# worm-privacy/proof-of-burn

Hardware: NVIDIA H100
Metric: main_proof_of_burn witnesses/sec (higher is better)
Workload: dtype u256 (BN254-Fr integer)

## Files before the change

proof-of-burn_b200/csrc/kernels.cuh:

```cuda
#pragma once
#include <cuda_runtime.h>
#include "vm_exec.h"
#include "cons_check.h"

using namespace pob;

namespace {

__constant__ uint64_t c_keccak_rc[24] = {
    0x0000000000000001ULL, 0x0000000000008082ULL, 0x800000000000808AULL, 0x8000000080008000ULL, 0x000000000000808BULL,
    0x0000000080000001ULL, 0x8000000080008081ULL, 0x8000000000008009ULL, 0x000000000000008AULL, 0x0000000000000088ULL,
    0x0000000080008009ULL, 0x000000008000000AULL, 0x000000008000808BULL, 0x800000000000008BULL, 0x8000000000008089ULL,
    0x8000000000008003ULL, 0x8000000000008002ULL, 0x8000000000000080ULL, 0x000000000000800AULL, 0x800000008000000AULL,
    0x8000000080008081ULL, 0x8000000000008080ULL, 0x0000000080000001ULL, 0x8000000080008008ULL};
__constant__ int c_keccak_rot[25] = {1, 10, 7, 11, 17, 18, 3, 5, 16, 8, 21, 24, 4, 15, 23, 19, 13, 12, 2, 20, 14, 22, 9, 6, 1};
__constant__ int c_keccak_inv_rot[25] = {0, 23, 17, 5, 11, 6, 22, 1, 8, 21, 0, 2, 16, 15, 19, 12, 7, 3, 4, 14, 18, 9, 20, 13, 10};

__device__ void absorb_warp(uint64_t *W, const AbsorbOp op) {
    const unsigned FULL = 0xffffffffu;
    const int lane = threadIdx.x & 31;
    const bool act = lane < 25;
    const int l = act ? lane : 0;
    uint64_t st = (act && op.s_idx != NONE_IDX) ? W[op.s_idx + l] : 0ull;
    if (lane < 17) st ^= W[op.blk_idx + lane];
// ... 219 lines not shown
                vm_exec_op(x, cur);
            }
        }
        for (uint32_t q = L.p_begin + gwarp; q < L.p_end; q += nwarp) poseidon_warp(x, a.poseidons[q], s_pk);
        { const uint32_t np = (L.p_end - L.p_begin) % nwarp, wv = (gwarp + nwarp - np) % nwarp;
          for (uint32_t w = L.w_begin + wv; w < L.w_end; w += nwarp) absorb_warp(U, a.absorbs[w]);
          const uint32_t nw2 = (np + (L.w_end - L.w_begin)) % nwarp, sv = (gwarp + nwarp - nw2) % nwarp;
          for (uint32_t q = L.s_begin + sv; q < L.s_end; q += nwarp) psum_warp(x, a.psums[q]); }
        if (inv_worker) {
            if (lv == a.ginv_level) {
                InvChain c;
                if (vm_ginv_start(x, a.ops, a.ginv_begin, a.inv_end, wid, NWK, c)) { inv_park(s_inv, INV_WORKERS, wt, c); inv_running = true; }
            } else if (inv_running) {
                InvChain c = inv_unpark(s_inv, INV_WORKERS, wt);
                if (inv_chain_steps(c, INV_STEPS)) { vm_ginv_finish(x, a.ops, a.ginv_begin, a.inv_end, wid, NWK, inv_chain_result(c)); inv_running = false; }
                else inv_park(s_inv, INV_WORKERS, wt, c);
            }
        }
        cluster_sync_all();
    }
    if (a.prof && inst == 0 && gt == 0) a.prof[a.n_levels] = clock64();
    if (inv_worker) {
        if (a.ginv_level >= a.n_levels) vm_inv_batch(x, a.ops, a.ginv_begin, a.inv_end, wid, NWK);
        else if (inv_running) {
            InvChain c = inv_unpark(s_inv, INV_WORKERS, wt);
            while (!inv_chain_steps(c, 64)) { }
            vm_ginv_finish(x, a.ops, a.ginv_begin, a.inv_end, wid, NWK, inv_chain_result(c));
        }
    }
    if (a.prof && inst == 0) { cluster_sync_all(); if (gt == 0) { a.prof[a.n_levels + 1] = clock64(); a.prof[a.n_levels + 2] = clock64(); } }
    __syncthreads();
    if (tid == 0 && s_status != STATUS_OK) atomicMin(a.status + inst, s_status);
    cluster_sync_all();
    if (gt == 0 && atomicAdd(a.status + inst, 0u) == STATUS_OK) a.status[inst] = 0u;
    for (uint32_t i = gt; i < a.n_outputs; i += GT) {
        uint64_t v[4]; vm_expand(a.out_codes[i], U, 0, a.val_base, a.konst, v);
        uint64_t *o = a.outputs + ((uint64_t)inst * a.n_outputs + i) * 4;
        o[0] = v[0]; o[1] = v[1]; o[2] = v[2]; o[3] = v[3];
    }
}

__device__ __forceinline__ void st128(uint64_t *p, uint64_t a, uint64_t b) { asm volatile("st.global.v2.b64 [%0], {%1, %2};" ::"l"(p), "l"(a), "l"(b)); }
__device__ __forceinline__ void st128cs(uint64_t *p, uint64_t a, uint64_t b) { asm volatile("st.global.cs.v2.b64 [%0], {%1, %2};" ::"l"(p), "l"(a), "l"(b)); }

struct ExpandArgs {
    const Tile *tiles; const Code *codes; const Fr *konst; const uint2 *round_desc;
    const uint64_t *stores; uint64_t store_stride; uint32_t val_base;
    uint64_t *const *wit;
    const uint32_t *inst;
    const uint32_t *status;
    uint32_t chunk_first;
    uint32_t tile0;
    uint32_t cs;
};

template <int T>
__global__ void __launch_bounds__(T) k_expand_round(const ExpandArgs a) {
    const uint32_t gi = a.inst[blockIdx.y];
    if (a.status[gi] != 0) return;
    const Tile t = a.tiles[blockIdx.x];
    const uint64_t *Ub = a.stores + (uint64_t)(gi - a.chunk_first) * a.store_stride + t.ubase;
    uint64_t *W = a.wit[blockIdx.y] + t.dst * 4;
    __shared__ __align__(16) uint2 sD[MAX_TILE_SIGNALS / 64];
    __shared__ __align__(16) uint64_t sWraw[ROUND_WORDS_SPAN + 3];
    __shared__ __align__(8) uint64_t s_bar;
    const uint32_t odd = (uint32_t)((reinterpret_cast<uintptr_t>(Ub) >> 3) & 1u);
    const uint32_t nd = (t.n + 63) >> 6, d_bytes = ((nd + 1) & ~1u) * 8u, w_bytes = (ROUND_WORDS_SPAN + 3) / 2 * 16u;
    if (threadIdx.x == 0) mbar_init(&s_bar, 1);
    __syncthreads();
    if (threadIdx.x == 0) {
        mbar_expect_tx(&s_bar, d_bytes + w_bytes);
        tma_load_1d(sD, a.round_desc + (t.code_off >> 6), d_bytes, &s_bar);
        tma_load_1d(sWraw, Ub - odd, w_bytes, &s_bar);
    }
    mbar_wait(&s_bar, 0);
    const uint64_t *sW = sWraw + odd;
#pragma unroll 8
    for (uint32_t u = threadIdx.x; u < 2 * t.n; u += T) {
        const uint32_t k = u >> 1;
        const uint2 d = sD[k >> 6];
        const uint32_t tt = k & 63, mode = d.y >> 16;
        uint32_t w = d.x & 0xffffu, b = tt;
        if (mode) {
            const uint32_t sidx = (mode - 1) * 64 + tt, g = sidx / 3, m = sidx - 3 * g;
            b = g; w = (m == 0) ? (d.x & 0xffffu) : (m == 1) ? (d.x >> 16) : (d.y & 0xffffu);
        }
        const uint64_t v = (u & 1u) ? 0ull : (sW[w] >> b) & 1ull;
        if (a.cs) st128cs(W + 2ull * u, v, 0); else st128(W + 2ull * u, v, 0);
    }
}

__global__ void __launch_bounds__(256, 3) k_expand_codes(const ExpandArgs a) {
    constexpr int UG = 4;
    const uint32_t gi = a.inst[blockIdx.x];
    if (a.status[gi] != 0) return;
    const Tile t = a.tiles[a.tile0 + blockIdx.y];
    const uint64_t *U = a.stores + (uint64_t)(gi - a.chunk_first) * a.store_stride;
    uint64_t *W = a.wit[blockIdx.x] + t.dst * 4;
    const uint64_t *Ub = U + t.ubase;
    __shared__ __align__(16) Code sC[TILE_SIGNALS + 4];
    __shared__ __align__(8) uint64_t s_bar;
    const uint32_t off4 = t.code_off & 3u, bytes = (((t.n + off4) * 4u) + 15u) & ~15u;
    if (threadIdx.x == 0) mbar_init(&s_bar, 1);
    __syncthreads();
    if (threadIdx.x == 0) { mbar_expect_tx(&s_bar, bytes); tma_load_1d(sC, a.codes + (t.code_off - off4), bytes, &s_bar); }
    mbar_wait(&s_bar, 0);
    const Code *c = sC + off4;
    const uint32_t n2 = 2 * t.n, h = threadIdx.x & 1u;
    for (uint32_t base = threadIdx.x; base < n2; base += 256 * UG) {
        uint64_t v[UG][2];
#pragma unroll
        for (int j = 0; j < UG; j++) {
            const uint32_t u = base + 256 * j;
            const Code cd = u < n2 ? c[u >> 1] : 0u;
            const uint32_t kind = code_kind(cd), p = code_payload(cd);
            v[j][0] = v[j][1] = 0;
            if (kind == K_VAL || kind == K_KONST) {
                const uint64_t *s = (kind == K_VAL) ? U + a.val_base + 4ull * p : reinterpret_cast<const uint64_t *>(a.konst + p);
                const ulonglong2 q = reinterpret_cast<const ulonglong2 *>(s)[h];
                v[j][0] = q.x; v[j][1] = q.y;
            } else if (!h) v[j][0] = (kind == K_BIT) ? (Ub[p >> 6] >> (p & 63)) & 1ull : p;
        }
#pragma unroll
        for (int j = 0; j < UG; j++) { const uint32_t u = base + 256 * j; if (u < n2) { if (a.cs) st128cs(W + 2ull * u, v[j][0], v[j][1]); else st128(W + 2ull * u, v[j][0], v[j][1]); } }
    }
}

__global__ void __launch_bounds__(256) k_digest(const uint64_t *wit, uint64_t n_signals, unsigned long long *out, const uint32_t *status) {
    if (status && *status != 0) return;
    uint64_t acc = 0;
    for (uint64_t i = (uint64_t)blockIdx.x * blockDim.x + threadIdx.x; i < n_signals; i += (uint64_t)gridDim.x * blockDim.x) {
        const ulonglong4 v = *reinterpret_cast<const ulonglong4 *>(wit + 4 * i);
        uint64_t h = (i + 1) * 0x9E3779B97F4A7C15ULL;
        h ^= v.x * 0xBF58476D1CE4E5B9ULL + v.y * 0x94D049BB133111EBULL + v.z * 0xD6E8FEB86659FD93ULL + v.w * 0xA0761D6478BD642FULL;
        h ^= h >> 29; h *= 0xBF58476D1CE4E5B9ULL; h ^= h >> 32;
        acc += h;
    }
    for (int o = 16; o > 0; o >>= 1) acc += __shfl_down_sync(0xffffffffu, acc, o);
    __shared__ uint64_t part[8];
    if ((threadIdx.x & 31) == 0) part[threadIdx.x >> 5] = acc;
    __syncthreads();
// ... 148 lines not shown
```

proof-of-burn_b200/csrc/pob_b200.cu:

```cuda
#include <cuda.h>
#include <cuda_runtime.h>
#include <fcntl.h>
#include <unistd.h>
#include <algorithm>
#include <chrono>
#include <condition_variable>
#include <cstdio>
#include <cstdlib>
#include <cstring>
#include <deque>
#include <mutex>
#include <stdexcept>
#include <string>
#include <thread>
#include <vector>
#include "../../include/pob_b200.h"
#include "compiler.h"
#include "kernels.cuh"
#include "ntt.cuh"
#include "r1cs.h"

using namespace pob;

static thread_local std::string g_err;
// ... 92 lines not shown
        busy[b] = true; next_b = (b + 1) % NB; return b;
    }
    void drain() { std::unique_lock<std::mutex> l(m); cv.wait(l, [this] { if (!q.empty()) return false; for (int i = 0; i < NB; i++) if (busy[i]) return false; return true; }); }
    static size_t header(uint8_t *o, uint64_t n) {
        uint32_t u32; uint64_t u64; Fr p = fr_p(); size_t k = 0;
        auto put = [&](const void *s, size_t b) { memcpy(o + k, s, b); k += b; };
        put("wtns", 4); u32 = 2; put(&u32, 4); u32 = 2; put(&u32, 4);
        u32 = 1; put(&u32, 4); u64 = 40; put(&u64, 8); u32 = 32; put(&u32, 4); put(p.l, 32); u32 = (uint32_t)n; put(&u32, 4);
        u32 = 2; put(&u32, 4); u64 = 32ull * n; put(&u64, 8);
        return k;
    }
    void send(const uint64_t *dwit, uint64_t n_signals, int fd) {
        CU(cudaSetDevice(device));
        if (fd >= 0) { uint8_t hd[80]; size_t hb = header(hd, n_signals); if (pwrite(fd, hd, hb, 0) != (ssize_t)hb) { std::lock_guard<std::mutex> l(m); io_err = true; } }
        const uint64_t total = 32ull * n_signals; const uint64_t nch = (total + bb - 1) / bb;
        for (uint64_t c = 0; c < nch; c++) {
            const uint64_t off = c * bb; const size_t bytes = (size_t)std::min<uint64_t>(bb, total - off);
            const int b = grab(); cudaStream_t s = cs[rr++ % NS];
            CU(cudaMemcpyAsync(buf[b], (const char *)dwit + off, bytes, cudaMemcpyDeviceToHost, s));
            CU(cudaEventRecord(ev[b], s));
            { std::lock_guard<std::mutex> l(m); q.push_back(Job{b, fd, 76 + off, bytes, c + 1 == nch}); }
            cv.notify_all();
            bytes_moved += bytes;
        }
        if (nch == 0 && fd >= 0) close(fd);
        for (int i = 1; i < NS; i++) { CU(cudaEventRecord(ev_join, cs[i])); CU(cudaStreamWaitEvent(cs[0], ev_join, 0)); }
    }
};

}

struct pob_handle {
    Program P; int device = 0; uint32_t n_sms = 0;
    Op *d_ops = nullptr; PsumOp *d_psums = nullptr; PoseidonOp *d_pos = nullptr; Fr *d_pos_konst = nullptr; AbsorbOp *d_abs = nullptr; Level *d_levels = nullptr; Code *d_aux = nullptr; Fr *d_konst = nullptr;
    Code *d_codes = nullptr; Tile *d_tiles = nullptr; Fr *d_invtab = nullptr; uint64_t *d_round_desc = nullptr;
    static const uint32_t RING = 2;
    uint32_t chunk = 0; uint64_t store_stride = 0; uint64_t *d_stores = nullptr; uint64_t *d_inputs = nullptr;
    std::vector<uint64_t *> slots;
    std::vector<VmSlot> slot_vm; size_t slot_bytes = 0; uint32_t n_compressed_slots = 0;
    std::vector<int64_t> slot_owner;
    std::vector<cudaEvent_t> slot_rel_ev; std::vector<uint8_t> slot_rel_pending;
    std::vector<uint32_t> last_status; uint32_t last_n = 0;
    uint32_t cap_n = 0; uint32_t *d_status = nullptr; uint64_t *d_outputs = nullptr; unsigned long long *d_digests = nullptr;
    uint64_t **d_witptr = nullptr; uint32_t *d_planinst = nullptr;
    uint32_t *h_status = nullptr; uint64_t *h_outputs = nullptr; uint64_t *h_digests = nullptr; uint64_t **h_witptr = nullptr; uint32_t *h_planinst = nullptr;
    uint64_t *d_staged = nullptr; uint32_t n_staged = 0;
    long long *d_prof = nullptr; std::string prof_path;
    uint32_t xgroup = 0;
    uint32_t n_round_tiles = 0;
    uint64_t *d_block_base = nullptr; uint32_t n_blocks = 0;
    uint32_t round_dyn_smem = 85 * 1024;
    uint32_t codes_dyn_smem = 24 * 1024;
    uint32_t round_threads = 256, codes_overlap = 0; bool serialize = false;
    int eval_threads = 512; uint32_t eval_cluster = 0, eval_prefetch = 0;
    uint32_t pos_konst_bytes = 0, levels_bytes = 0, eval_smem = 0;
    bool skip_eval = false;
    uint32_t expand_cs = 0, eval_l2_mb = 0;
    cudaStream_t s_eval = nullptr, s_exp = nullptr, s_exp2 = nullptr, s_h2d = nullptr;
    cudaEvent_t ev_eval_done[RING] = {nullptr, nullptr}, ev_exp_done[RING] = {nullptr, nullptr}, ev_h2d[RING] = {nullptr, nullptr},
                ev_start = nullptr, ev_end = nullptr, ev_tmp = nullptr, ev_fork = nullptr, ev_join = nullptr;
    std::vector<cudaEvent_t> ev_pool; size_t ev_used = 0;
    struct Group { uint32_t begin, end, chunk; cudaEvent_t t0, t1; };
    struct Batch {
        bool active = false, async = false, staged = false, expand = false, digest = false;
        const uint64_t *inputs = nullptr; uint32_t n = 0, nchunks = 0, next_eval = 0, next_group = 0, acq_pos = 0;
        std::vector<uint32_t> plan, slot;
        std::vector<uint8_t> st;
        std::vector<uint32_t> group_of;
        std::vector<Group> groups; std::vector<uint32_t> chunk_gend;
        std::vector<cudaEvent_t> e0, e1, est;
        pob_timing T{};
    } B;
    Exporter *exporter = nullptr;
    pob_timing timing{};
    struct DevCons {
        bool ready = false; ConsView flat{}, round{}; Fr *konst = nullptr; uint64_t *bases = nullptr; uint32_t n_blocks = 0;
        unsigned long long *rep = nullptr; std::vector<void *> allocs; pob_check_report info{};
    } cons, r1cs;
    struct DevNtt { bool ready = false; uint32_t log_n = 0; NttTables t{}; std::vector<void *> allocs; } ntt;
};

static void cons_info(const Program &P, pob_check_report *r) {
    memset(r, 0, sizeof *r);
    const uint64_t nb = P.round_block_sig.size();
    auto count = [&](const ConsSet &S, uint64_t mult) {
        r->n_constraints += mult * (S.eq.size() / 2 + S.kc.size());
        for (const ConsR1 &q : S.r1) { if (r1_hint(q)) r->n_hints += mult; else { r->n_constraints += mult; if (q.na) r->n_nonlinear += mult; } }
    };
    count(P.cons_flat, 1); count(P.cons_round, nb);
    std::vector<uint8_t> seen(P.n_signals, 0);
    auto mark = [&](const ConsSet &S, uint64_t base) {
        for (uint32_t i : S.eq) seen[base + i] = 1;
        for (const ConsTerm &t : S.kc) seen[base + t.idx] = 1;
        for (const ConsTerm &t : S.terms) if (t.idx != CONS_ONE) seen[base + t.idx] = 1;
    };
    mark(P.cons_flat, 0);
    for (uint64_t b : P.round_block_sig) mark(P.cons_round, b);
    for (uint8_t v : seen) r->signals_read += v;
    r->first_failed = ~0ull;
}
static ConsView upload_cons(pob_handle::DevCons &C, const ConsSet &S) {
    ConsView v{};
    auto up = [&](const void *src, size_t bytes) { void *d = nullptr; CU(cudaMalloc(&d, std::max<size_t>(16, bytes))); if (bytes) CU(cudaMemcpy(d, src, bytes, cudaMemcpyHostToDevice)); C.allocs.push_back(d); return d; };
    v.eq = (const uint32_t *)up(S.eq.data(), S.eq.size() * 4); v.n_eq = S.eq.size() / 2;
    v.kc = (const ConsTerm *)up(S.kc.data(), S.kc.size() * sizeof(ConsTerm)); v.n_kc = S.kc.size();
    v.r1 = (const ConsR1 *)up(S.r1.data(), S.r1.size() * sizeof(ConsR1)); v.n_r1 = S.r1.size();
// ... 60 lines not shown
    uint64_t *stores = h->d_stores + (size_t)r * E * h->store_stride;
    EvalArgs ea{h->d_ops, h->d_abs, h->d_pos, h->d_pos_konst, h->d_psums, h->d_levels, (uint32_t)P.levels.size(), P.inv_begin, P.ginv_begin, P.inv_end, h->d_aux, h->d_konst, h->d_invtab,
                h->d_codes + P.out_code_off, P.n_outputs, P.n_inputs, P.val_base, stores, h->store_stride, d_in,
                h->d_status + first, h->d_outputs + (size_t)first * no * 4, (c == 0) ? h->d_prof : nullptr, h->pos_konst_bytes, h->levels_bytes, h->eval_prefetch, P.ginv_level};
    CU(cudaEventRecord(B.e0[c], h->s_eval));
    {
        uint32_t C = h->eval_cluster;
        if (C == 0) { C = 8; while (C > 1 && cnt * C > h->n_sms) C >>= 1; }
        cudaLaunchConfig_t cfg{}; cudaLaunchAttribute at[1];
        cfg.gridDim = dim3(cnt * C); cfg.blockDim = dim3((unsigned)h->eval_threads); cfg.dynamicSmemBytes = h->eval_smem; cfg.stream = h->s_eval;
        at[0].id = cudaLaunchAttributeClusterDimension; at[0].val.clusterDim.x = C; at[0].val.clusterDim.y = 1; at[0].val.clusterDim.z = 1;
        cfg.attrs = at; cfg.numAttrs = 1;
        B.T.eval_clusters |= 1u << C;
        if (h->skip_eval && c >= R) CU(cudaMemsetAsync(h->d_status + first, 0, (size_t)cnt * 4, h->s_eval));
        else switch (h->eval_threads) {
        case 256: CU(cudaLaunchKernelEx(&cfg, k_eval<256>, ea)); break;
        case 512: CU(cudaLaunchKernelEx(&cfg, k_eval<512>, ea)); break;
        default: CU(cudaLaunchKernelEx(&cfg, k_eval<1024>, ea)); break;
        }
    }
    CU(cudaEventRecord(B.e1[c], h->s_eval));
    CU(cudaEventRecord(h->ev_eval_done[r], h->s_eval));
    B.T.eval_launches++;
    CU(cudaMemcpyAsync(h->h_status + first, h->d_status + first, (size_t)cnt * 4, cudaMemcpyDeviceToHost, h->s_eval));
    B.T.d2h_bytes += (uint64_t)cnt * 4;
    if (P.n_outputs) { CU(cudaMemcpyAsync(h->h_outputs + (size_t)first * no * 4, h->d_outputs + (size_t)first * no * 4, (size_t)cnt * no * 32, cudaMemcpyDeviceToHost, h->s_eval)); B.T.d2h_bytes += (uint64_t)cnt * no * 32; }
    CU(cudaEventRecord(B.est[c], h->s_eval));
    const uint32_t g0 = c ? B.chunk_gend[c - 1] : 0;
    if (B.chunk_gend[c] == g0) CU(cudaEventRecord(h->ev_exp_done[r], h->s_eval));
}

static void enqueue_group(pob_handle *h, uint32_t g) {
    pob_handle::Batch &B = h->B; const Program &P = h->P;
    const pob_handle::Group &G = B.groups[g];
    const uint32_t E = h->chunk, R = pob_handle::RING, r = G.chunk % R, gc = G.end - G.begin;
    CU(cudaStreamWaitEvent(h->s_exp, h->ev_eval_done[r], 0));
    for (uint32_t k = G.begin; k < G.end; k++) {
        const uint32_t s = B.slot[k];
        if (h->slot_rel_pending[s]) { CU(cudaStreamWaitEvent(h->s_exp, h->slot_rel_ev[s], 0)); h->slot_rel_pending[s] = 0; }
        h->slot_owner[s] = (int64_t)B.plan[k];
    }
    ExpandArgs xa{h->d_tiles, h->d_codes, h->d_konst, reinterpret_cast<const uint2 *>(h->d_round_desc), h->d_stores + (size_t)r * E * h->store_stride, h->store_stride, P.val_base,
                  h->d_witptr + G.begin, h->d_planinst + G.begin, h->d_status, G.chunk * E, 0, h->expand_cs};
    CU(cudaEventRecord(G.t0, h->s_exp));
    const uint32_t n_round = h->n_round_tiles, n_code = (uint32_t)P.tiles.size() - n_round;
    const bool fork = h->codes_overlap && n_round && n_code;
    cudaStream_t s_codes = fork ? h->s_exp2 : h->s_exp;
    auto launch_codes = [&]() {
        xa.tile0 = n_round;
        k_expand_codes<<<dim3(gc, n_code), 256, h->codes_dyn_smem, s_codes>>>(xa);
        B.T.other_launches++;
    };
    if (fork) { CU(cudaEventRecord(h->ev_fork, h->s_exp)); CU(cudaStreamWaitEvent(h->s_exp2, h->ev_fork, 0)); if (h->codes_overlap == 2) launch_codes(); }
    if (n_round) {
        xa.tile0 = 0;
        if (h->round_threads == 128) k_expand_round<128><<<dim3(n_round, gc), 128, h->round_dyn_smem, h->s_exp>>>(xa);
        else if (h->round_threads == 512) k_expand_round<512><<<dim3(n_round, gc), 512, h->round_dyn_smem, h->s_exp>>>(xa);
        else if (h->round_threads == 1024) k_expand_round<1024><<<dim3(n_round, gc), 1024, h->round_dyn_smem, h->s_exp>>>(xa);
        else k_expand_round<256><<<dim3(n_round, gc), 256, h->round_dyn_smem, h->s_exp>>>(xa);
    }
    if (n_code && !(fork && h->codes_overlap == 2)) launch_codes();
    if (fork) { CU(cudaEventRecord(h->ev_join, h->s_exp2)); CU(cudaStreamWaitEvent(h->s_exp, h->ev_join, 0)); }
    CU(cudaEventRecord(G.t1, h->s_exp));
    B.T.expand_launches++;
    if (B.digest) for (uint32_t k = G.begin; k < G.end; k++) {
        k_digest<<<h->n_sms * 8, 256, 0, h->s_exp>>>(h->slots[B.slot[k]], P.n_signals, h->d_digests + B.plan[k], h->d_status + B.plan[k]);
        B.T.other_launches++;
    }
    if (!B.async) for (uint32_t k = G.begin; k < G.end; k++) B.st[k] = 2;
    if (g + 1 == B.chunk_gend[G.chunk]) {
        CU(cudaEventRecord(h->ev_exp_done[r], h->s_exp));
        if (h->serialize) CU(cudaStreamWaitEvent(h->s_eval, h->ev_exp_done[r], 0));
    }
}

static bool group_slots_free(const pob_handle *h, uint32_t g) {
    const pob_handle::Batch &B = h->B; const uint32_t ns = (uint32_t)h->slots.size();
    for (uint32_t k = B.groups[g].begin; k < B.groups[g].end; k++) if (k >= ns && B.st[k - ns] != 2) return false;
    return true;
}
static void advance(pob_handle *h) {
    pob_handle::Batch &B = h->B; const uint32_t R = pob_handle::RING, ng = (uint32_t)B.groups.size();
    for (;;) {
        bool progressed = false;
        if (B.next_eval < B.nchunks && (B.next_eval < R || B.next_group >= B.chunk_gend[B.next_eval - R])) { enqueue_eval(h, B.next_eval++); progressed = true; }
        if (B.next_group < ng && B.groups[B.next_group].chunk < B.next_eval && group_slots_free(h, B.next_group)) { enqueue_group(h, B.next_group++); progressed = true; }
        if (!progressed) break;
    }
    CU(cudaGetLastError());
}

static int begin_batch(pob_handle *h, const uint64_t *inputs, uint32_t n, uint32_t flags, const uint32_t *retain, uint32_t n_retain, bool async, const char *who) {
    const bool staged = (flags & POB_RUN_INPUTS_STAGED) != 0, digest = (flags & POB_RUN_DIGEST) != 0;
    const bool expand = async || (flags & (POB_RUN_EXPAND | POB_RUN_DIGEST)) != 0 || retain != nullptr;
    if (h->B.active) return fail(POB_E_BUSY, std::string(who) + ": a batch is in flight on this handle (pob_finish it first)");
    if (staged ? (h->n_staged < n) : (inputs == nullptr && h->P.n_inputs)) return fail(POB_E_BAD_ARG, std::string(who) + ": no inputs");
    const uint32_t ns = (uint32_t)h->slots.size();
    if (retain) {
        if (n_retain > ns) return fail(POB_E_RANGE, std::string(who) + ": more retained instances than witness slots");
        for (uint32_t k = 0; k < n_retain; k++) if (retain[k] >= n || (k && retain[k] <= retain[k - 1])) return fail(POB_E_BAD_ARG, std::string(who) + ": retain[] must be strictly ascending instance indices");
    } else if (expand && !async && n > ns && !(flags & (POB_RUN_DIGEST | POB_RUN_DISCARD)))
        return fail(POB_E_RANGE, std::string(who) + ": n exceeds the resident witness slots; earlier witnesses would be overwritten unread -- use pob_submit/pob_acquire/pob_release, a retain list, POB_RUN_DIGEST or POB_RUN_DISCARD");
    CU(cudaSetDevice(h->device));
    ensure_batch_buffers(h, n);
    pob_handle::Batch &B = h->B;
    B = pob_handle::Batch();
    B.async = async; B.staged = staged; B.expand = expand; B.digest = digest; B.inputs = inputs; B.n = n;
    const uint32_t E = h->chunk;
    B.nchunks = (n + E - 1) / E;
    const uint32_t X = async ? std::max<uint32_t>(1, std::min(h->xgroup, ns / 2 ? ns / 2 : 1)) : h->xgroup;
    if (expand) {
        if (retain) B.plan.assign(retain, retain + n_retain);
// ... 18 lines not shown
    std::fill(h->slot_owner.begin(), h->slot_owner.end(), (int64_t)-1);
    std::fill(h->slot_rel_pending.begin(), h->slot_rel_pending.end(), (uint8_t)0);
    h->last_n = 0; h->last_status.clear();
    CU(cudaEventRecord(h->ev_start, h->s_eval));
    if (np) {
        CU(cudaMemcpyAsync(h->d_witptr, h->h_witptr, (size_t)np * sizeof(uint64_t *), cudaMemcpyHostToDevice, h->s_eval));
        CU(cudaMemcpyAsync(h->d_planinst, h->h_planinst, (size_t)np * 4, cudaMemcpyHostToDevice, h->s_eval));
    }
    if (digest) CU(cudaMemsetAsync(h->d_digests, 0, (size_t)n * 8, h->s_eval));
    CU(cudaEventRecord(h->ev_tmp, h->s_eval));
    CU(cudaStreamWaitEvent(h->s_h2d, h->ev_tmp, 0));
    B.active = true;
    advance(h);
    return POB_OK;
}

static int finish_batch(pob_handle *h, uint32_t *status, uint64_t *outputs, uint64_t *digests) {
    pob_handle::Batch &B = h->B; const Program &P = h->P;
    const uint32_t n = B.n; const size_t no = std::max<uint32_t>(1, P.n_outputs);
    for (auto &s : B.st) s = 2;
    advance(h);
    if (B.next_eval != B.nchunks || B.next_group != B.groups.size()) throw std::runtime_error("internal: batch did not drain");
    CU(cudaEventRecord(h->ev_tmp, h->s_eval));
    CU(cudaStreamWaitEvent(h->s_exp, h->ev_tmp, 0));
    if (B.digest) { CU(cudaMemcpyAsync(h->h_digests, h->d_digests, (size_t)n * 8, cudaMemcpyDeviceToHost, h->s_exp)); B.T.d2h_bytes += (uint64_t)n * 8; }
    CU(cudaEventRecord(h->ev_end, h->s_exp));
    CU(cudaStreamSynchronize(h->s_exp)); CU(cudaStreamSynchronize(h->s_eval)); CU(cudaStreamSynchronize(h->s_h2d));
    CU(cudaGetLastError());
    if (status) memcpy(status, h->h_status, (size_t)n * 4);
    if (outputs && P.n_outputs) memcpy(outputs, h->h_outputs, (size_t)n * no * 32);
    if (B.digest && digests) memcpy(digests, h->h_digests, (size_t)n * 8);
    pob_timing &T = B.T;
    CU(cudaEventElapsedTime(&T.total_ms, h->ev_start, h->ev_end));
    for (uint32_t c = 0; c < B.nchunks; c++) { float ms = 0; CU(cudaEventElapsedTime(&ms, B.e0[c], B.e1[c])); T.eval_ms += ms; }
    for (auto &G : B.groups) { float ms = 0; CU(cudaEventElapsedTime(&ms, G.t0, G.t1)); T.expand_ms += ms; }
    if (h->d_prof) {
        std::vector<long long> st(P.levels.size() + 3);
        CU(cudaMemcpy(st.data(), h->d_prof, st.size() * sizeof(long long), cudaMemcpyDeviceToHost));
        if (FILE *f = fopen(h->prof_path.c_str(), "w")) {
            for (size_t l = 0; l + 1 < st.size(); l++) {
                if (l < P.levels.size()) fprintf(f, "level %zu ops %u absorbs %u poseidons %u cycles %lld\n", l, P.levels[l].t_end - P.levels[l].t_begin, P.levels[l].w_end - P.levels[l].w_begin, P.levels[l].p_end - P.levels[l].p_begin, st[l + 1] - st[l]);
                else if (l == P.levels.size()) fprintf(f, "inverse-batch(table) ops %u cycles %lld\n", P.ginv_begin - P.inv_begin, st[l + 1] - st[l]);
                else fprintf(f, "inverse-batch(generic) ops %u cycles %lld\n", P.inv_end - P.ginv_begin, st[l + 1] - st[l]);
            }
            fclose(f);
        }
    }
    h->timing = T; h->last_n = n; h->last_status.assign(h->h_status, h->h_status + n);
    B.active = false;
    return POB_OK;
}
static void abort_batch(pob_handle *h) {
    cudaDeviceSynchronize(); cudaGetLastError();
    h->B.active = false; h->last_n = 0; h->last_status.clear();
    std::fill(h->slot_owner.begin(), h->slot_owner.end(), (int64_t)-1);
}

extern "C" {

const char *pob_last_error(void) { return g_err.c_str(); }
const char *pob_version(void) {
#ifdef POB_TUNING
    return "pob_b200 0.2 (sm_90a, TUNING build)";
#else
    return "pob_b200 0.2 (sm_90a)";
#endif
}

const char *pob_input_schema(const char *main_name, int *nparams) {
    if (!main_name) return nullptr;
    return main_input_schema(main_name, nparams);
}

int pob_layout_info(const char *main_name, const uint64_t *params, int nparams, int hcreate, pob_desc *out) {
    if (!main_name || !out || (nparams > 0 && !params)) return fail(POB_E_BAD_ARG, "pob_layout_info: null argument");
    try { Program P = compile_circuit(main_name, params_vec(params, nparams), flag_hcreate(hcreate), false, flag_opt(hcreate)); fill_desc(P, out); }
    catch (const std::exception &e) { return fail(POB_E_COMPILE, e.what()); }
    return POB_OK;
}

int pob_write_components(const char *main_name, const uint64_t *params, int nparams, int hcreate, const char *path, uint64_t *n_components) {
    if (!main_name || !path || (nparams > 0 && !params)) return fail(POB_E_BAD_ARG, "pob_write_components: null argument");
    try { uint64_t n = write_components(main_name, params_vec(params, nparams), flag_hcreate(hcreate), path); if (n_components) *n_components = n; }
    catch (const std::exception &e) { return fail(POB_E_COMPILE, e.what()); }
    return POB_OK;
}

int pob_write_r1cs(const char *main_name, const uint64_t *params, int nparams, int hcreate, const char *path, pob_r1cs_desc *out) {
    if (!main_name || !out || (nparams > 0 && !params)) return fail(POB_E_BAD_ARG, "pob_write_r1cs: null argument");
    try {
        const RowPlan R = build_row_plan(main_name, params_vec(params, nparams), flag_hcreate(hcreate), flag_opt(hcreate));
        memset(out, 0, sizeof *out);
        out->n_wires = R.n_wires; out->n_pub_out = R.n_outputs; out->n_pub_in = 0; out->n_prv_in = R.n_inputs; out->n_labels = R.n_labels;
        out->n_constraints = R.n_rows(); out->n_nonlinear = R.n_nonlinear; out->n_terms = R.n_terms; out->file_bytes = R.file_bytes();
        if (path) write_r1cs(R, path);
    } catch (const R1csIoError &e) { return fail(POB_E_IO, std::string("pob_write_r1cs: ") + e.what()); }
    catch (const std::exception &e) { return fail(POB_E_COMPILE, e.what()); }
    return POB_OK;
}

void pob_destroy(pob_handle *h) {
    if (!h) return;
    cudaSetDevice(h->device);
    delete h->exporter; h->exporter = nullptr;
    for (void *p : h->cons.allocs) cudaFree(p);
    for (void *p : h->r1cs.allocs) cudaFree(p);
    for (void *p : h->ntt.allocs) cudaFree(p);
    if (h->s_eval) cudaStreamSynchronize(h->s_eval);
    if (h->s_exp2) cudaStreamSynchronize(h->s_exp2);
    if (h->s_exp) cudaStreamSynchronize(h->s_exp);
    if (h->s_h2d) cudaStreamSynchronize(h->s_h2d);
    for (void *p : {(void *)h->d_ops, (void *)h->d_psums, (void *)h->d_pos, (void *)h->d_pos_konst, (void *)h->d_abs, (void *)h->d_levels, (void *)h->d_aux, (void *)h->d_konst, (void *)h->d_codes,
                    (void *)h->d_tiles, (void *)h->d_invtab, (void *)h->d_round_desc, (void *)h->d_stores, (void *)h->d_inputs, (void *)h->d_status,
                    (void *)h->d_outputs, (void *)h->d_digests, (void *)h->d_witptr, (void *)h->d_planinst, (void *)h->d_staged, (void *)h->d_prof, (void *)h->d_block_base})
        if (p) cudaFree(p);
    if (!h->slot_vm.empty()) {
        const DriverVmm &D = vmm();
        cudaDeviceSynchronize();
        for (const VmSlot &s : h->slot_vm) {
            if (s.mapped) D.unmap(s.va, h->slot_bytes);
            if (s.va) D.addressFree(s.va, h->slot_bytes);
            if (s.mem) D.release(s.mem);
        }
    }
    for (void *p : {(void *)h->h_status, (void *)h->h_outputs, (void *)h->h_digests, (void *)h->h_witptr, (void *)h->h_planinst}) if (p) cudaFreeHost(p);
    for (cudaEvent_t e : h->ev_pool) cudaEventDestroy(e);
    for (cudaEvent_t e : h->slot_rel_ev) cudaEventDestroy(e);
    for (uint32_t r = 0; r < pob_handle::RING; r++) {
        if (h->ev_eval_done[r]) cudaEventDestroy(h->ev_eval_done[r]);
        if (h->ev_exp_done[r]) cudaEventDestroy(h->ev_exp_done[r]);
        if (h->ev_h2d[r]) cudaEventDestroy(h->ev_h2d[r]);
    }
    for (cudaEvent_t e : {h->ev_start, h->ev_end, h->ev_tmp, h->ev_fork, h->ev_join}) if (e) cudaEventDestroy(e);
    for (cudaStream_t s : {h->s_h2d, h->s_eval, h->s_exp, h->s_exp2}) if (s) cudaStreamDestroy(s);
    delete h;
}

int pob_create(const char *main_name, const uint64_t *params, int nparams, int hcreate, int device, uint32_t max_slots, pob_handle **out) {
    if (!main_name || !out || (nparams > 0 && !params)) return fail(POB_E_BAD_ARG, "pob_create: null argument");
    *out = nullptr;
    int ndev = 0;
    if (cudaGetDeviceCount(&ndev) != cudaSuccess || ndev == 0) return fail(POB_E_NO_DEVICE, "pob_create: no CUDA device (this library has no CPU path)");
    if (device < 0 || device >= ndev) return fail(POB_E_NO_DEVICE, "pob_create: device index out of range");
    pob_handle *h = new pob_handle(); h->device = device;
    try { h->P = compile_circuit(main_name, params_vec(params, nparams), flag_hcreate(hcreate), false, flag_opt(hcreate)); }
    catch (const std::exception &e) { delete h; return fail(POB_E_COMPILE, e.what()); }
    try {
        const Program &P = h->P;
        CU(cudaSetDevice(device));
        { int v = 0; CU(cudaDeviceGetAttribute(&v, cudaDevAttrMultiProcessorCount, device)); h->n_sms = (uint32_t)v; }
        h->d_ops = upload(P.ops); h->d_psums = upload(P.psums); h->d_pos = upload(P.poseidons); h->d_pos_konst = upload(P.pos_konst); h->d_abs = upload(P.absorbs); h->d_levels = upload(P.levels); h->d_aux = upload(P.aux);
        h->pos_konst_bytes = (uint32_t)(P.pos_konst.size() * sizeof(Fr)); h->levels_bytes = (uint32_t)(std::max<size_t>(1, P.levels.size()) * sizeof(Level));
        h->d_konst = upload(P.konst);
        { std::vector<Code> cd = P.codes; cd.resize(cd.size() + 8, 0); h->d_codes = upload(cd); }
        if (const char *v = tune_env("POB_TILE_FILTER")) {
            std::vector<Tile> sub; for (const Tile &t : P.tiles) if ((atoi(v) == 1) == (t.pad != 0)) sub.push_back(t);
            h->P.tiles = sub;
        }
        h->d_tiles = upload(h->P.tiles);
        for (const Tile &t : h->P.tiles) if (t.pad) h->n_round_tiles++;
        { std::vector<uint64_t> bases; for (const Tile &t : P.tiles) if (t.pad && t.code_off == 0) bases.push_back(t.dst);
          std::sort(bases.begin(), bases.end()); h->n_blocks = (uint32_t)bases.size(); h->d_block_base = upload(bases); }
        h->d_invtab = upload(build_inverse_table());
        { std::vector<uint64_t> rd = P.round_desc; rd.resize(rd.size() + 2, 0); h->d_round_desc = upload(rd); }
        int pr_least = 0, pr_greatest = 0; CU(cudaDeviceGetStreamPriorityRange(&pr_least, &pr_greatest));
        CU(cudaStreamCreateWithPriority(&h->s_eval, cudaStreamNonBlocking, pr_greatest));
        CU(cudaStreamCreateWithPriority(&h->s_h2d, cudaStreamNonBlocking, pr_greatest));
// ... 24 lines not shown
        size_t gran = 0; CUD(D.granularity(&gran, &mprop, CU_MEM_ALLOC_GRANULARITY_RECOMMENDED));
        const size_t vbytes = (wbytes + gran - 1) / gran * gran;
        const uint64_t ring_bytes_per_inst = pob_handle::RING * (h->store_stride * 8 + (uint64_t)P.n_inputs * 32);
        uint64_t budget = (uint64_t)(free_b * 0.8);
        uint64_t nslots = budget > chunk * ring_bytes_per_inst ? (budget - chunk * ring_bytes_per_inst) / vbytes : 0;
        if (max_slots && nslots > max_slots) nslots = max_slots;
        if (nslots > 4096) nslots = 4096;
        if (nslots == 0) throw std::runtime_error("not even one witness slot fits in free HBM");
        h->chunk = chunk;
        CU(cudaMalloc(&h->d_stores, (size_t)pob_handle::RING * chunk * h->store_stride * 8));
        CU(cudaMalloc(&h->d_inputs, std::max<size_t>(32, (size_t)pob_handle::RING * chunk * P.n_inputs * 32)));
        h->slot_bytes = vbytes;
        CUmemAccessDesc acc{}; acc.location = mprop.location; acc.flags = CU_MEM_ACCESS_FLAGS_PROT_READWRITE;
        for (uint64_t s = 0; s < nslots; s++) {
            CUmemGenericAllocationHandle mem = 0;
            const CUresult r = D.create(&mem, vbytes, &mprop, 0);
            if (r == CUDA_ERROR_OUT_OF_MEMORY && s > 0) break;
            if (r == CUDA_ERROR_OUT_OF_MEMORY) throw std::runtime_error("not even one witness slot fits in free HBM (cuMemCreate)");
            if (r != CUDA_SUCCESS) throw std::runtime_error("cuMemCreate: CUresult " + std::to_string((int)r));
            h->slot_vm.push_back(VmSlot{}); VmSlot &m = h->slot_vm.back(); m.mem = mem;
            CUD(D.reserve(&m.va, vbytes, gran, 0, 0));
            CUD(D.map(m.va, vbytes, 0, m.mem, 0)); m.mapped = true;
            CUD(D.setAccess(m.va, vbytes, &acc, 1));
            CUmemAllocationProp got{}; CUD(D.properties(&got, m.mem));
            if (got.allocFlags.compressionType == CU_MEM_ALLOCATION_COMP_GENERIC) h->n_compressed_slots++;
            h->slots.push_back(reinterpret_cast<uint64_t *>(m.va));
        }
        nslots = h->slots.size();
        h->xgroup = (uint32_t)std::min<uint64_t>(std::min<uint64_t>(nslots, chunk), std::max<uint64_t>(16, (100ull << 30) / wbytes));
        if (const char *v = tune_env("POB_EVAL_THREADS")) h->eval_threads = atoi(v);
        if (const char *v = tune_env("POB_EVAL_CLUSTER")) h->eval_cluster = (uint32_t)std::max(0, std::min(8, atoi(v)));
        if (const char *v = tune_env("POB_EVAL_PREFETCH")) h->eval_prefetch = (uint32_t)(atoi(v) != 0);
        if (const char *v = tune_env("POB_SKIP_EVAL")) h->skip_eval = atoi(v) != 0;
        if (const char *v = tune_env("POB_EXPAND_CS")) h->expand_cs = (uint32_t)(atoi(v) != 0);
        if (const char *v = tune_env("POB_EVAL_L2_MB")) h->eval_l2_mb = (uint32_t)std::max(0, atoi(v));
        if (h->eval_threads != 256 && h->eval_threads != 512) h->eval_threads = 1024;
        h->eval_smem = h->pos_konst_bytes + h->levels_bytes + INV_WORKERS * INV_PARK_WORDS * 4u;
        if (h->eval_smem > 200 * 1024) throw std::runtime_error("the Poseidon constant table, the level table and the parked inversions do not fit in shared memory");
        CU(cudaFuncSetAttribute(k_eval<256>, cudaFuncAttributeMaxDynamicSharedMemorySize, (int)h->eval_smem));
        CU(cudaFuncSetAttribute(k_eval<512>, cudaFuncAttributeMaxDynamicSharedMemorySize, (int)h->eval_smem));
        CU(cudaFuncSetAttribute(k_eval<1024>, cudaFuncAttributeMaxDynamicSharedMemorySize, (int)h->eval_smem));
        if (const char *v = tune_env("POB_SERIALIZE")) h->serialize = atoi(v) != 0;
        if (const char *v = tune_env("POB_EXPAND_SMEM_KB")) h->round_dyn_smem = (uint32_t)atoi(v) * 1024u;
        if (const char *v = tune_env("POB_EXPAND_THREADS")) h->round_threads = (uint32_t)atoi(v);
        if (const char *v = tune_env("POB_CODES_OVERLAP")) h->codes_overlap = (uint32_t)atoi(v);
        if (const char *v = tune_env("POB_CODES_SMEM_KB")) h->codes_dyn_smem = (uint32_t)atoi(v) * 1024u;
        CU(cudaFuncSetAttribute(k_expand_codes, cudaFuncAttributeMaxDynamicSharedMemorySize, (int)h->codes_dyn_smem));
        if (h->round_dyn_smem > 48 * 1024) {
            CU(cudaFuncSetAttribute(k_expand_round<128>, cudaFuncAttributeMaxDynamicSharedMemorySize, (int)h->round_dyn_smem));
            CU(cudaFuncSetAttribute(k_expand_round<256>, cudaFuncAttributeMaxDynamicSharedMemorySize, (int)h->round_dyn_smem));
            CU(cudaFuncSetAttribute(k_expand_round<512>, cudaFuncAttributeMaxDynamicSharedMemorySize, (int)h->round_dyn_smem));
            CU(cudaFuncSetAttribute(k_expand_round<1024>, cudaFuncAttributeMaxDynamicSharedMemorySize, (int)h->round_dyn_smem));
        }
        if (const char *v = tune_env("POB_EXPAND_GROUP")) h->xgroup = (uint32_t)std::max(1, std::min<int>(atoi(v), (int)std::min<uint64_t>(nslots, chunk)));
        if (h->eval_l2_mb) {
            const size_t ring = (size_t)pob_handle::RING * chunk * h->store_stride * 8, carve = (size_t)h->eval_l2_mb << 20;
            CU(cudaDeviceSetLimit(cudaLimitPersistingL2CacheSize, carve));
            cudaDeviceProp prop; CU(cudaGetDeviceProperties(&prop, device));
            cudaStreamAttrValue av{};
            av.accessPolicyWindow.base_ptr = h->d_stores;
            av.accessPolicyWindow.num_bytes = std::min<size_t>(ring, (size_t)prop.accessPolicyMaxWindowSize);
            av.accessPolicyWindow.hitRatio = (float)std::min(1.0, (double)carve / (double)av.accessPolicyWindow.num_bytes);
            av.accessPolicyWindow.hitProp = cudaAccessPropertyPersisting; av.accessPolicyWindow.missProp = cudaAccessPropertyStreaming;
            CU(cudaStreamSetAttribute(h->s_eval, cudaStreamAttributeAccessPolicyWindow, &av));
        }
        h->slot_owner.assign(nslots, -1); h->slot_rel_pending.assign(nslots, 0);
        for (uint64_t s = 0; s < nslots; s++) { cudaEvent_t e; CU(cudaEventCreateWithFlags(&e, cudaEventDisableTiming)); h->slot_rel_ev.push_back(e); }
    } catch (const std::exception &e) {
        std::string m = e.what(); pob_destroy(h);
        return fail(m.find("slot") != std::string::npos ? POB_E_NO_MEMORY : POB_E_CUDA, "pob_create: " + m);
    }
    *out = h; return POB_OK;
}

int pob_witness_map(const pob_handle *h, uint32_t *map) {
    if (!h || !map) return fail(POB_E_BAD_ARG, "pob_witness_map: null argument");
    if (!h->P.opt_level) return fail(POB_E_BAD_ARG, "pob_witness_map: the handle produces the full --O0 witness (identity map)");
    memcpy(map, h->P.witness_map.data(), h->P.witness_map.size() * 4);
    return POB_OK;
}

int pob_describe(const pob_handle *h, pob_desc *out) {
    if (!h || !out) return fail(POB_E_BAD_ARG, "pob_describe: null argument");
    fill_desc(h->P, out); out->n_slots = (uint32_t)h->slots.size(); out->chunk = h->chunk; out->expand_group = h->xgroup;
    out->n_compressed_slots = h->n_compressed_slots; return POB_OK;
}

void *pob_alloc_pinned(uint64_t bytes) { void *p = nullptr; if (cudaMallocHost(&p, bytes ? bytes : 1) != cudaSuccess) { g_err = "cudaMallocHost failed"; return nullptr; } return p; }
void pob_free_pinned(void *p) { if (p) cudaFreeHost(p); }

int pob_stage_inputs(pob_handle *h, const uint64_t *inputs, uint32_t n) {
    if (!h || !inputs || n == 0) return fail(POB_E_BAD_ARG, "pob_stage_inputs: bad argument");
    if (h->B.active) return fail(POB_E_BUSY, "pob_stage_inputs: a batch is in flight");
    try {
        CU(cudaSetDevice(h->device));
        if (h->d_staged) { cudaFree(h->d_staged); h->d_staged = nullptr; h->n_staged = 0; }
        size_t bytes = std::max<size_t>(32, (size_t)n * h->P.n_inputs * 32);
        CU(cudaMalloc(&h->d_staged, bytes));
        if (h->P.n_inputs) CU(cudaMemcpy(h->d_staged, inputs, (size_t)n * h->P.n_inputs * 32, cudaMemcpyHostToDevice));
        h->n_staged = n;
    } catch (const std::exception &e) { return fail(POB_E_CUDA, e.what()); }
    return POB_OK;
}

static int run_batch_impl(pob_handle *h, const uint64_t *inputs, uint32_t n, uint32_t flags, const uint32_t *retain, uint32_t n_retain,
                          uint32_t *status, uint64_t *outputs, uint64_t *digests, const char *who) {
// ... 407 lines not shown
```

proof-of-burn_b200/csrc/program.h:

```cpp
#pragma once
#include <stdint.h>
#include <string>
#include <vector>
#include "fr_hd.h"

namespace pob {

typedef uint32_t Code;
enum : uint32_t { K_CONST = 0, K_BIT = 1, K_VAL = 2, K_KONST = 3 };
POB_HD uint32_t code_kind(Code c) { return c >> 30; }
POB_HD uint32_t code_payload(Code c) { return c & 0x3fffffffu; }
POB_HD Code c_const(uint32_t v) { return v; }
POB_HD Code c_bit(uint32_t u64idx, uint32_t bit) { return (1u << 30) | (u64idx << 6) | bit; }
POB_HD Code c_val(uint32_t slot) { return (2u << 30) | slot; }
POB_HD Code c_konst(uint32_t idx) { return (3u << 30) | idx; }
static const uint32_t MAX_STORE_U64 = 1u << 24;

enum Opc : uint32_t {
    OP_FMA = 1,
    OP_ISZ = 2,
    OP_INV = 3,
    OP_DIV = 4,
    OP_MOD = 5,
    OP_PACK8 = 6,
    OP_CHK_EQ = 7,
    OP_CHK_RANGE = 8,
    OP_GTC = 9,
    OP_SELSUM = 10,
};
struct Op { uint32_t opc_dst; Code a, b, c; };
POB_HD uint32_t op_opc(const Op &o) { return o.opc_dst >> 26; }
POB_HD uint32_t op_dst(const Op &o) { return o.opc_dst & 0x3ffffffu; }

static const uint32_t NONE_IDX = 0xffffffffu;
struct AbsorbOp { uint32_t s_idx, blk_idx, out_idx, pad; };
enum : uint32_t { RW = 238, RW_X5 = 25, RW_DD = 45, RW_TH = 65, RW_RP = 90, RW_CH = 162, RW_RC = 237, RW_OUT = 238,
                  ROUND_WORDS_SPAN = 263, ABSORB_WORDS = 25 + 24 * 238, ROUND_SIGNALS = 102656 };
POB_HD uint32_t rw_x5(int i, int k) { return RW_X5 + 4 * i + k; }
POB_HD uint32_t rw_dd(int i, int k) { return RW_DD + 4 * i + k; }
POB_HD uint32_t rw_th(int l) { return RW_TH + l; }
POB_HD uint32_t rw_rp(int i, int k) { return RW_RP + 3 * i + k; }
POB_HD uint32_t rw_ch(int l, int k) { return RW_CH + 3 * l + k; }
POB_HD uint32_t rw_out(int l) { return RW_OUT + l; }

struct PoseidonOp { uint32_t t, in_aux, base, koff, q0, q1; };
static const uint32_t POS_SEGMENTS = 16;
struct PosLayout { uint32_t t, rp, F1, PB, SB, LB, total, kC, kS, kM, kP, ktotal; };
POB_HD PosLayout pos_layout(uint32_t t) {
    PosLayout L; L.t = t; L.rp = (t == 3) ? 57u : (t == 4) ? 56u : 60u;
    L.F1 = t; L.PB = 21 * t; L.SB = L.PB + L.rp * (4 + t); L.LB = L.SB + 15 * t; L.total = L.LB + 3 * t + 1;
    L.kC = 0; L.kS = t * 8 + L.rp; L.kM = L.kS + L.rp * (2 * t - 1); L.kP = L.kM + t * t; L.ktotal = L.kP + t * t;
    return L;
}
POB_HD uint32_t pos_steps(const PosLayout &L) { return L.rp + 9; }
POB_HD uint32_t pos_state_off(const PosLayout &L, uint32_t q) {
    if (q == 0) return 0;
    if (q <= 4) return L.F1 + 5 * L.t * (q - 1) + 4 * L.t;
    if (q < 5 + L.rp) return L.PB + (q - 5) * (4 + L.t) + 4;
    return L.SB + 5 * L.t * (q - 5 - L.rp) + 4 * L.t;
}

POB_HD uint32_t pos_step_begin(const PosLayout &L, uint32_t q) {
    if (q == 0) return 0;
    if (q <= 4) return L.F1 + 5 * L.t * (q - 1);
    if (q < 5 + L.rp) return L.PB + (q - 5) * (4 + L.t);
    if (q < L.rp + 8) return L.SB + 5 * L.t * (q - 5 - L.rp);
    return q == L.rp + 8 ? L.LB : L.total;
}

struct PsumOp { uint32_t aux0, n, dst; Code x0; };

struct Level { uint32_t t_begin, t_end, w_begin, w_end, p_begin, p_end, s_begin, s_end; };

struct Tile { uint64_t dst; uint32_t n, code_off, ubase, pad; };
static const uint32_t TILE_SIGNALS = 8192;
static const uint32_t LAYOUT_TILE_SIGNALS = 4096;
static const uint32_t MAX_TILE_SIGNALS = 32768;

struct ConsTerm { uint32_t idx, coef; };
enum : uint32_t { CC_POS = 0, CC_NEG = 1, CC_KONST = 2, CC_RCBIT = 3 };
POB_HD uint32_t cc_kind(uint32_t c) { return c >> 30; }
POB_HD uint32_t cc_payload(uint32_t c) { return c & 0x3fffffffu; }
struct ConsR1 { uint32_t off; uint16_t nc_hint; uint8_t na, nb; };
POB_HD uint32_t r1_nc(const ConsR1 &r) { return r.nc_hint & 0x7fffu; }
POB_HD bool r1_hint(const ConsR1 &r) { return (r.nc_hint >> 15) != 0; }
struct ConsSet {
    std::vector<uint32_t> eq;
    std::vector<ConsTerm> kc;
    std::vector<ConsR1> r1;
    std::vector<ConsTerm> terms;
    uint64_t n_records() const { return eq.size() / 2 + kc.size() + r1.size(); }
};

struct Program {
    std::string main_name;
    std::vector<Fr> params;
    bool hcreate = false;
    uint64_t n_signals = 0;
    uint32_t n_outputs = 0, n_inputs = 0;
    std::string input_schema;
    uint32_t n_words = 0;
    uint32_t val_base = 0;
    uint32_t n_vals = 0;
    uint64_t store_u64() const { return (uint64_t)val_base + 4ull * n_vals; }
    std::vector<Op> ops;
    uint32_t inv_begin = 0, ginv_begin = 0, inv_end = 0;
    uint32_t ginv_level = 0xffffffffu;
    std::vector<AbsorbOp> absorbs;
    std::vector<PoseidonOp> poseidons;
    std::vector<PsumOp> psums;
    std::vector<Fr> pos_konst;
    std::vector<Level> levels;
    std::vector<Code> aux;
    std::vector<Fr> konst;
    std::vector<Code> codes;
    std::vector<Tile> tiles;
    std::vector<uint64_t> round_desc;
    bool has_constraints = false;
    ConsSet cons_flat, cons_round;
    std::vector<Fr> cons_konst;
    std::vector<uint64_t> round_block_sig;
    int opt_level = 0;
    uint64_t n_signals_o0 = 0;
    std::vector<uint32_t> witness_map;
    uint32_t out_code_off = ROUND_SIGNALS + 1;
    uint64_t n_round_blocks = 0, n_flat_signals = 0;
};

}
```

Measured before the change: 564.9.

## Split round tiles into sorted work units and add optional persistent round-expand kernel

Round tiles are split into smaller units, 2048 signals at optimized level by default, sorted by destination, and the default non-persistent k_expand_round now launches over these units. An opt-in persistent kernel claims units through a global atomic ticket and double-buffers the TMA loads of the round words. It also keeps the whole descriptor table resident in shared memory. The aim is better load balance and overlap of loads with bit-expansion stores, at the cost of more, smaller blocks and atomic contention if enabled.

```diff
diff --git a/proof-of-burn_b200/csrc/kernels.cuh b/proof-of-burn_b200/csrc/kernels.cuh
--- a/proof-of-burn_b200/csrc/kernels.cuh
+++ b/proof-of-burn_b200/csrc/kernels.cuh
@@ -295,6 +295,12 @@
     uint32_t chunk_first;
     uint32_t tile0;
     uint32_t cs;
+    const Tile *units;
+    uint32_t n_units_w;
+    uint32_t desc_bytes;
+    uint64_t n_units;
+    unsigned long long *claim;
+    unsigned long long ticket0;
 };
 
 template <int T>
@@ -330,6 +336,60 @@
         }
         const uint64_t v = (u & 1u) ? 0ull : (sW[w] >> b) & 1ull;
         if (a.cs) st128cs(W + 2ull * u, v, 0); else st128(W + 2ull * u, v, 0);
+    }
+}
+
+struct RoundUnit { uint64_t *W; uint32_t n, d0, odd, pad; };
+template <int T>
+__global__ void __launch_bounds__(T) k_expand_round_persistent(const ExpandArgs a) {
+    extern __shared__ __align__(128) uint8_t dyn_smem[];
+    constexpr uint32_t RWB = ROUND_WORDS_SPAN + 3, W_BYTES = RWB / 2 * 16u;
+    const uint2 *sD = reinterpret_cast<const uint2 *>(dyn_smem);
+    uint64_t *sWb = reinterpret_cast<uint64_t *>(dyn_smem + a.desc_bytes);
+    __shared__ __align__(8) uint64_t s_bar[2];
+    __shared__ RoundUnit s_u[2];
+    auto claim = [&](uint32_t b, bool first) {
+        for (;;) {
+            const unsigned long long q = atomicAdd(a.claim, 1ull) - a.ticket0;
+            if (q >= a.n_units) { s_u[b].n = 0; return; }
+            const uint32_t w = (uint32_t)(q / a.n_units_w), j = (uint32_t)(q - (uint64_t)w * a.n_units_w);
+            const uint32_t gi = a.inst[w];
+            if (a.status[gi] != 0) continue;
+            const Tile t = a.units[j];
+            const uint64_t *Ub = a.stores + (uint64_t)(gi - a.chunk_first) * a.store_stride + t.ubase;
+            const uint32_t odd = (uint32_t)((reinterpret_cast<uintptr_t>(Ub) >> 3) & 1u);
+            s_u[b] = RoundUnit{a.wit[w] + t.dst * 4, t.n, t.code_off >> 6, odd, 0};
+            mbar_expect_tx(&s_bar[b], W_BYTES + (first ? a.desc_bytes : 0u));
+            if (first) tma_load_1d(dyn_smem, a.round_desc, a.desc_bytes, &s_bar[b]);
+            tma_load_1d(sWb + b * RWB, Ub - odd, W_BYTES, &s_bar[b]);
+            return;
+        }
+    };
+    if (threadIdx.x == 0) { mbar_init(&s_bar[0], 1); mbar_init(&s_bar[1], 1); }
+    __syncthreads();
+    if (threadIdx.x == 0) claim(0, true);
+    __syncthreads();
+    for (uint32_t it = 0;; it++) {
+        const uint32_t b = it & 1u;
+        const RoundUnit u = s_u[b];
+        if (u.n == 0) break;
+        if (threadIdx.x == 0) claim(b ^ 1u, false);
+        mbar_wait(&s_bar[b], (it >> 1) & 1u);
+        const uint64_t *sW = sWb + b * RWB + u.odd;
+#pragma unroll 8
+        for (uint32_t h = threadIdx.x; h < 2 * u.n; h += T) {
+            const uint32_t k = h >> 1;
+            const uint2 d = sD[u.d0 + (k >> 6)];
+            const uint32_t tt = k & 63, mode = d.y >> 16;
+            uint32_t w = d.x & 0xffffu, bit = tt;
+            if (mode) {
+                const uint32_t sidx = (mode - 1) * 64 + tt, g = sidx / 3, m = sidx - 3 * g;
+                bit = g; w = (m == 0) ? (d.x & 0xffffu) : (m == 1) ? (d.x >> 16) : (d.y & 0xffffu);
+            }
+            const uint64_t v = (h & 1u) ? 0ull : (sW[w] >> bit) & 1ull;
+            if (a.cs) st128cs(u.W + 2ull * h, v, 0); else st128(u.W + 2ull * h, v, 0);
+        }
+        __syncthreads();
     }
 }
 
diff --git a/proof-of-burn_b200/csrc/pob_b200.cu b/proof-of-burn_b200/csrc/pob_b200.cu
--- a/proof-of-burn_b200/csrc/pob_b200.cu
+++ b/proof-of-burn_b200/csrc/pob_b200.cu
@@ -168,6 +168,9 @@
     uint32_t round_dyn_smem = 85 * 1024;
     uint32_t codes_dyn_smem = 24 * 1024;
     uint32_t round_threads = 256, codes_overlap = 0; bool serialize = false;
+    bool round_persistent = false;
+    uint32_t unit_signals = MAX_TILE_SIGNALS, n_units_w = 0, round_grid = 0, persist_dyn_smem = 0, round_desc_bytes = 0;
+    Tile *d_units = nullptr; unsigned long long *d_claim = nullptr, claim_ticket = 0;
     int eval_threads = 512; uint32_t eval_cluster = 0, eval_prefetch = 0;
     uint32_t pos_konst_bytes = 0, levels_bytes = 0, eval_smem = 0;
     bool skip_eval = false;
@@ -334,12 +337,21 @@
         B.T.other_launches++;
     };
     if (fork) { CU(cudaEventRecord(h->ev_fork, h->s_exp)); CU(cudaStreamWaitEvent(h->s_exp2, h->ev_fork, 0)); if (h->codes_overlap == 2) launch_codes(); }
-    if (n_round) {
-        xa.tile0 = 0;
-        if (h->round_threads == 128) k_expand_round<128><<<dim3(n_round, gc), 128, h->round_dyn_smem, h->s_exp>>>(xa);
-        else if (h->round_threads == 512) k_expand_round<512><<<dim3(n_round, gc), 512, h->round_dyn_smem, h->s_exp>>>(xa);
-        else if (h->round_threads == 1024) k_expand_round<1024><<<dim3(n_round, gc), 1024, h->round_dyn_smem, h->s_exp>>>(xa);
-        else k_expand_round<256><<<dim3(n_round, gc), 256, h->round_dyn_smem, h->s_exp>>>(xa);
+    if (n_round && h->round_persistent) {
+        xa.units = h->d_units; xa.n_units_w = h->n_units_w; xa.desc_bytes = h->round_desc_bytes;
+        xa.n_units = (uint64_t)gc * h->n_units_w; xa.claim = h->d_claim; xa.ticket0 = h->claim_ticket;
+        if (h->round_threads == 128) k_expand_round_persistent<128><<<h->round_grid, 128, h->persist_dyn_smem, h->s_exp>>>(xa);
+        else if (h->round_threads == 512) k_expand_round_persistent<512><<<h->round_grid, 512, h->persist_dyn_smem, h->s_exp>>>(xa);
+        else k_expand_round_persistent<256><<<h->round_grid, 256, h->persist_dyn_smem, h->s_exp>>>(xa);
+        CU(cudaGetLastError());
+        h->claim_ticket += xa.n_units + h->round_grid;
+    } else if (n_round) {
+        ExpandArgs ra = xa; ra.tiles = h->d_units; ra.tile0 = 0;
+        const dim3 grid(h->n_units_w, gc);
+        if (h->round_threads == 128) k_expand_round<128><<<grid, 128, h->round_dyn_smem, h->s_exp>>>(ra);
+        else if (h->round_threads == 512) k_expand_round<512><<<grid, 512, h->round_dyn_smem, h->s_exp>>>(ra);
+        else if (h->round_threads == 1024) k_expand_round<1024><<<grid, 1024, h->round_dyn_smem, h->s_exp>>>(ra);
+        else k_expand_round<256><<<grid, 256, h->round_dyn_smem, h->s_exp>>>(ra);
     }
     if (n_code && !(fork && h->codes_overlap == 2)) launch_codes();
     if (fork) { CU(cudaEventRecord(h->ev_join, h->s_exp2)); CU(cudaStreamWaitEvent(h->s_exp, h->ev_join, 0)); }
@@ -464,6 +476,9 @@
 }
 static void abort_batch(pob_handle *h) {
     cudaDeviceSynchronize(); cudaGetLastError();
+    unsigned long long v = 0;
+    if (h->d_claim && cudaMemcpy(&v, h->d_claim, sizeof v, cudaMemcpyDeviceToHost) == cudaSuccess) h->claim_ticket = v;
+    cudaGetLastError();
     h->B.active = false; h->last_n = 0; h->last_status.clear();
     std::fill(h->slot_owner.begin(), h->slot_owner.end(), (int64_t)-1);
 }
@@ -524,7 +539,7 @@
     if (h->s_h2d) cudaStreamSynchronize(h->s_h2d);
     for (void *p : {(void *)h->d_ops, (void *)h->d_psums, (void *)h->d_pos, (void *)h->d_pos_konst, (void *)h->d_abs, (void *)h->d_levels, (void *)h->d_aux, (void *)h->d_konst, (void *)h->d_codes,
                     (void *)h->d_tiles, (void *)h->d_invtab, (void *)h->d_round_desc, (void *)h->d_stores, (void *)h->d_inputs, (void *)h->d_status,
-                    (void *)h->d_outputs, (void *)h->d_digests, (void *)h->d_witptr, (void *)h->d_planinst, (void *)h->d_staged, (void *)h->d_prof, (void *)h->d_block_base})
+                    (void *)h->d_outputs, (void *)h->d_digests, (void *)h->d_witptr, (void *)h->d_planinst, (void *)h->d_staged, (void *)h->d_prof, (void *)h->d_block_base, (void *)h->d_units, (void *)h->d_claim})
         if (p) cudaFree(p);
     if (!h->slot_vm.empty()) {
         const DriverVmm &D = vmm();
@@ -655,6 +670,36 @@
             CU(cudaFuncSetAttribute(k_expand_round<512>, cudaFuncAttributeMaxDynamicSharedMemorySize, (int)h->round_dyn_smem));
             CU(cudaFuncSetAttribute(k_expand_round<1024>, cudaFuncAttributeMaxDynamicSharedMemorySize, (int)h->round_dyn_smem));
         }
+        if (const char *v = tune_env("POB_ROUND_PERSISTENT")) h->round_persistent = atoi(v) != 0;
+        if (P.opt_level) h->unit_signals = REDUCED_ROUND_UNIT_SIGNALS;
+        if (const char *v = tune_env("POB_ROUND_UNIT")) { const int s = atoi(v); if (s >= 128 && s % 128 == 0 && s <= (int)MAX_TILE_SIGNALS) h->unit_signals = (uint32_t)s; }
+        if (h->n_round_tiles) {
+            std::vector<Tile> units;
+            for (uint32_t i = 0; i < h->n_round_tiles; i++) {
+                const Tile &t = h->P.tiles[i];
+                for (uint32_t o = 0; o < t.n; o += h->unit_signals) { Tile u = t; u.dst += o; u.code_off += o; u.n = std::min(h->unit_signals, t.n - o); units.push_back(u); }
+            }
+            std::sort(units.begin(), units.end(), [](const Tile &x, const Tile &y) { return x.dst < y.dst; });
+            h->n_units_w = (uint32_t)units.size(); h->d_units = upload(units);
+        }
+        if (h->round_persistent && h->n_round_tiles) {
+            CU(cudaMalloc(&h->d_claim, sizeof(unsigned long long))); CU(cudaMemset(h->d_claim, 0, sizeof(unsigned long long)));
+            h->round_desc_bytes = (uint32_t)((P.round_desc.size() * 8 + 15) & ~size_t(15));
+            const uint32_t need = h->round_desc_bytes + 2 * (ROUND_WORDS_SPAN + 3) * 8;
+            h->persist_dyn_smem = std::max(h->round_dyn_smem, need);
+            if (const char *v = tune_env("POB_ROUND_CTAS_PER_SM")) {
+                const int k = atoi(v);
+                h->persist_dyn_smem = std::max(need, (k <= 1 ? 120u : k == 2 ? 85u : k == 3 ? 56u : 40u) * 1024u);
+            }
+            if (h->persist_dyn_smem > 200 * 1024) throw std::runtime_error("the KeccakfRound descriptor table does not fit in shared memory");
+            int k = 0;
+            for (auto f : {k_expand_round_persistent<128>, k_expand_round_persistent<256>, k_expand_round_persistent<512>})
+                CU(cudaFuncSetAttribute(f, cudaFuncAttributeMaxDynamicSharedMemorySize, (int)h->persist_dyn_smem));
+            const int T = h->round_threads == 128 ? 128 : h->round_threads == 512 ? 512 : 256;
+            CU(cudaOccupancyMaxActiveBlocksPerMultiprocessor(&k, T == 128 ? k_expand_round_persistent<128> : T == 512 ? k_expand_round_persistent<512> : k_expand_round_persistent<256>, T, h->persist_dyn_smem));
+            if (k < 1) throw std::runtime_error("k_expand_round_persistent cannot be resident");
+            h->round_grid = h->n_sms * (uint32_t)k;
+        }
         if (const char *v = tune_env("POB_EXPAND_GROUP")) h->xgroup = (uint32_t)std::max(1, std::min<int>(atoi(v), (int)std::min<uint64_t>(nslots, chunk)));
         if (h->eval_l2_mb) {
             const size_t ring = (size_t)pob_handle::RING * chunk * h->store_stride * 8, carve = (size_t)h->eval_l2_mb << 20;
diff --git a/proof-of-burn_b200/csrc/program.h b/proof-of-burn_b200/csrc/program.h
--- a/proof-of-burn_b200/csrc/program.h
+++ b/proof-of-burn_b200/csrc/program.h
@@ -76,6 +76,7 @@
 static const uint32_t TILE_SIGNALS = 8192;
 static const uint32_t LAYOUT_TILE_SIGNALS = 4096;
 static const uint32_t MAX_TILE_SIGNALS = 32768;
+static const uint32_t REDUCED_ROUND_UNIT_SIGNALS = 2048;
 
 struct ConsTerm { uint32_t idx, coef; };
 enum : uint32_t { CC_POS = 0, CC_NEG = 1, CC_KONST = 2, CC_RCBIT = 3 };
```

New measurement: 564.9 (median of 6 runs). Within noise of the previous version (-0.0%).
